# WeebLabs/DSPi

Measured on NVIDIA H100. Metric: audio samples/sec (whole box) at 65536ch x 10-band EQ, 96 kHz; % HBM roofline, higher is better.
Workload: dtype f32

## Files before the change

dspi_b200/csrc/engine.cu:

```cuda
#include <cstdarg>
#include <cstdio>
#include <cstdlib>
#include <cstring>
#include <algorithm>
#include <new>
#include <utility>
#include <vector>
#include <sched.h>
#include <unistd.h>
#include <sys/syscall.h>

#include "eq_kernels.cuh"
#include "eq_jit.h"

namespace {

thread_local char g_err[512] = "";

int fail(int code, const char *fmt, ...)
{
    va_list ap;
    va_start(ap, fmt);
    vsnprintf(g_err, sizeof(g_err), fmt, ap);
    va_end(ap);
// ... 143 lines not shown
    int ndev = 0;
    if (cudaGetDeviceCount(&ndev) != cudaSuccess || ndev == 0) { cudaGetLastError(); return fail(DSPI_ENODEV, "no CUDA device (there is no CPU fallback)"); }
    if (desc->device < 0 || desc->device >= ndev) return fail(DSPI_ENODEV, "device %d out of range (%d visible)", desc->device, ndev);
    int major = 0;
    CU_OK(cudaDeviceGetAttribute(&major, cudaDevAttrComputeCapabilityMajor, desc->device));
    if (major != 9) return fail(DSPI_ENODEV, "device %d has compute capability %d.x; the kernels are built for sm_90a only", desc->device, major);
    if (!encode_fn()) return fail(DSPI_ENODEV, "driver does not export cuTensorMapEncodeTiled");
    CU_OK(cudaSetDevice(desc->device));

    dspi_eq *e = new (std::nothrow) dspi_eq();
    if (!e) return fail(DSPI_ENOMEM, "host allocation failed");
    memset(e, 0, sizeof(*e));
    e->desc = *desc;
    e->sig_dirty = true;
    const bool q28 = desc->arith == DSPI_ARITH_Q28;
    e->cpl = 2;
    if (const char *v = getenv("DSPI_F32_CPL")) e->cpl = atoi(v) == 1 ? 1 : 2;
    if (q28) e->cpl = 1;
    e->rows = 32u * e->cpl;
    e->n_groups = (desc->n_channels + e->rows - 1) / e->rows;
    e->c_pad = e->n_groups * e->rows;
    e->aos_elem = q28 ? sizeof(dspi_biquad_q28) : sizeof(dspi_biquad_f32);

    cudaError_t err;
    const size_t aos_bytes = (size_t)e->c_pad * DSPI_MAX_BANDS * e->aos_elem;
    const size_t coef_bytes = q28 ? (size_t)e->n_groups * DSPI_MAX_BANDS * 20 * 32 * 4 : (size_t)e->c_pad * DSPI_MAX_BANDS * 8 * 4;
    if ((err = cudaStreamCreateWithFlags(&e->stream, cudaStreamNonBlocking)) != cudaSuccess) goto cuda_fail;
    if ((err = cudaStreamCreateWithFlags(&e->s_h2d, cudaStreamNonBlocking)) != cudaSuccess) goto cuda_fail;
    if ((err = cudaStreamCreateWithFlags(&e->s_d2h, cudaStreamNonBlocking)) != cudaSuccess) goto cuda_fail;
    if ((err = cudaEventCreateWithFlags(&e->ev_begin, cudaEventDisableTiming)) != cudaSuccess) goto cuda_fail;
    for (int i = 0; i < kHostBufs; i++) {
        if ((err = cudaStreamCreateWithFlags(&e->s_k[i], cudaStreamNonBlocking)) != cudaSuccess) goto cuda_fail;
// ... 133 lines not shown
    const cuuint64_t gstride[1] = { (cuuint64_t)ld * 4 };
    const cuuint32_t box[2] = { 32, e->rows };
    const cuuint32_t estr[2] = { 1, 1 };
    const CUtensorMapDataType dt = e->desc.arith == DSPI_ARITH_Q28 ? CU_TENSOR_MAP_DATA_TYPE_INT32 : CU_TENSOR_MAP_DATA_TYPE_FLOAT32;
    CUresult r = encode_fn()(out, dt, 2, d_samples, gdim, gstride, box, estr, CU_TENSOR_MAP_INTERLEAVE_NONE, CU_TENSOR_MAP_SWIZZLE_128B,
                             CU_TENSOR_MAP_L2_PROMOTION_L2_256B, CU_TENSOR_MAP_FLOAT_OOB_FILL_NONE);
    if (r != CUDA_SUCCESS) return fail(DSPI_ECUDA, "cuTensorMapEncodeTiled failed (%d) for T=%u ld=%u rows=%u", (int)r, T, ld, n_rows);
    return DSPI_OK;
}

static int refresh_kernel_choice(dspi_eq *e)
{
    e->sig_dirty = false;
    e->jit = nullptr;
    if (e->desc.arith == DSPI_ARITH_Q28) { snprintf(e->kinfo, sizeof(e->kinfo), "aot q28 cascade (K2)"); return DSPI_OK; }
    if (e->cpl != 2) { snprintf(e->kinfo, sizeof(e->kinfo), "aot scalar generic (DSPI_F32_CPL=1)"); return DSPI_OK; }
    const uint32_t C = e->desc.n_channels, nb = e->desc.n_bands;
    const int nbt = nb <= 10 ? 10 : 12;
    const uint32_t step = C > 2048 ? C / 2048 : 1;
    const uint32_t cnt = (C + step - 1) / step;
    std::vector<uint64_t> w(cnt);
    CU_OK(cudaMemcpy2DAsync(w.data(), 8, e->d_modes_eff ? e->d_modes_eff : e->d_modes, (size_t)step * 8, 8, cnt, cudaMemcpyDeviceToHost, e->stream));
    CU_OK(cudaStreamSynchronize(e->stream));
    const uint64_t mask = (1ull << (4 * nb)) - 1;
    for (auto &x : w) x &= mask;
    std::vector<uint64_t> sorted(w);
    std::sort(sorted.begin(), sorted.end());
    uint64_t best = 0;
    uint32_t best_n = 0;
    for (uint32_t i = 0; i < cnt;) {
        uint32_t j = i;
        while (j < cnt && sorted[j] == sorted[i]) j++;
        if (j - i > best_n) { best_n = j - i; best = sorted[i]; }
        i = j;
    }
    uint64_t tdf2 = 0;
    for (int b = 0; b < nbt; b++) tdf2 |= (uint64_t)dspi::kModeTdf2 << (4 * b);
    const unsigned pct = (unsigned)(100ull * best_n / cnt);
    if (best == tdf2 && (int)nb == nbt) {
        snprintf(e->kinfo, sizeof(e->kinfo), "aot straight-line biquad (%u%% of sampled channels are all-TDF2)", pct);
        return DSPI_OK;
    }
    bool force = false;
    const bool on = dspi::jit::enabled_by_env(&force);
    const char *why = nullptr;
    if (!on) why = "DSPI_JIT=0";
    else if (best == 0) why = "all bands bypassed";
    else if (2 * best_n < cnt) why = "no dominant topology vector";
    else if (!force && C < 1024) why = "engine below 1024 channels (DSPI_JIT=force overrides)";
    if (why) {
        snprintf(e->kinfo, sizeof(e->kinfo), "aot generic column path (%s)", why);
        return DSPI_OK;
    }
    char msg[256] = "";
    e->jit = dspi::jit::acquire(best, e->desc.arith == DSPI_ARITH_F32_FUSED, nbt, e->desc.device, msg, sizeof(msg));
    if (e->jit) snprintf(e->kinfo, sizeof(e->kinfo), "jit sig=0x%llx nb=%d (%u%% of sampled channels)", (unsigned long long)best, nbt, pct);
    else snprintf(e->kinfo, sizeof(e->kinfo), "aot generic column path (jit unavailable: %.200s)", msg);
    return DSPI_OK;
}

static int launch_eq(dspi_eq *e, void *d_samples, uint32_t T, uint32_t ld, uint32_t g0, uint32_t ng, uint32_t n_rows, cudaStream_t stream)
{
    dspi::EqLaunch a;
    memset(&a, 0, sizeof(a));
    const bool tma_ok = (ld % 4 == 0) && (((uintptr_t)d_samples & 15) == 0);
    if (tma_ok) {
        if (e->tm_ptr != d_samples || e->tm_T != T || e->tm_ld != ld || e->tm_rows != n_rows) {
            int rc = make_tmap(e, d_samples, T, ld, n_rows, &e->tmap);
            if (rc) return rc;
            e->tm_ptr = d_samples; e->tm_T = T; e->tm_ld = ld; e->tm_rows = n_rows;
        }
        a.tmap = e->tmap;
// ... 21 lines not shown
    if (q28) err = dspi::launch_eq_q28(a, stream);
    else if (e->jit && !(a.dbg & 12u)) {
        char msg[200] = "";
        err = dspi::jit::launch(e->jit, a, stream, msg, sizeof(msg));
        if (err != cudaSuccess) return fail(DSPI_ECUDA, "%s", msg);
    } else err = dspi::launch_eq_f32(a, e->desc.arith == DSPI_ARITH_F32_FUSED, e->cpl, stream);
    if (err != cudaSuccess) return fail(DSPI_ECUDA, "EQ kernel launch: %s", cudaGetErrorString(err));
    e->launches++;
    return DSPI_OK;
}

}

namespace dspi {

void *eq_aos_mirror(dspi_eq *e) { return e->d_aos; }

static int remask(dspi_eq *e, cudaStream_t s)
{
    if (!e->d_skip) return DSPI_OK;
    if (e->desc.arith == DSPI_ARITH_Q28) {
        CU_OK(launch_skip_q28((int32_t *)e->d_coef, e->d_skip, e->desc.n_channels, s));
        e->launches++;
        return DSPI_OK;
    }
    if (!e->d_modes_eff) {
        CU_OK(cudaMalloc(&e->d_modes_eff, (size_t)e->c_pad * 8));
        CU_OK(cudaMemsetAsync(e->d_modes_eff, 0, (size_t)e->c_pad * 8, s));
    }
    CU_OK(launch_mask_modes(e->d_modes, e->d_skip, e->d_modes_eff, e->desc.n_channels, s));
// ... 52 lines not shown
int eq_state_imported(dspi_eq *e, cudaStream_t s)
{
    e->sig_dirty = true;
    return remask(e, s);
}

int eq_process_on(dspi_eq *e, void *d_samples, uint32_t T, uint32_t ld, cudaStream_t s)
{
    if (T == 0) return DSPI_OK;
    return launch_eq(e, d_samples, T, ld, 0, e->n_groups, e->desc.n_channels, s);
}

int eq_process_range_on(dspi_eq *e, void *d_rows, uint32_t T, uint32_t ld, uint32_t ch0, uint32_t n, cudaStream_t s)
{
    if (T == 0 || n == 0) return DSPI_OK;
    if (ch0 % e->rows) return fail(DSPI_EINVAL, "first channel %u is not a multiple of the engine's group size %u", ch0, e->rows);
    CU_OK(cudaSetDevice(e->desc.device));
    return launch_eq(e, d_rows, T, ld, ch0 / e->rows, (n + e->rows - 1) / e->rows, n, s);
}

}

extern "C" {

int dspi_eq_kernel_info(dspi_eq *e, char *buf, size_t cap)
{
    if (!e || !buf || cap == 0) return fail(DSPI_EINVAL, "null argument");
    CU_OK(cudaSetDevice(e->desc.device));
    if (e->sig_dirty) {
        int rc = refresh_kernel_choice(e);
        if (rc) return rc;
// ... 5 lines not shown
int dspi_eq_process_device(dspi_eq *e, void *d_samples, uint32_t T, uint32_t ld)
{
    if (!e || !d_samples) return fail(DSPI_EINVAL, "null argument");
    if (T == 0) return DSPI_OK;
    if (ld < T) return fail(DSPI_EINVAL, "row stride %u < T %u", ld, T);
    CU_OK(cudaSetDevice(e->desc.device));
    return launch_eq(e, d_samples, T, ld, 0, e->n_groups, e->desc.n_channels, e->stream);
}

int dspi_eq_process_device_range(dspi_eq *e, void *d_rows, uint32_t T, uint32_t ld, uint32_t ch0, uint32_t n)
{
    if (!e || !d_rows) return fail(DSPI_EINVAL, "null argument");
    if (T == 0 || n == 0) return DSPI_OK;
    if (ld < T) return fail(DSPI_EINVAL, "row stride %u < T %u", ld, T);
    if ((uint64_t)ch0 + n > e->desc.n_channels) return fail(DSPI_ERANGE, "channels [%u, %u) outside engine of %u", ch0, ch0 + n, e->desc.n_channels);
    if (ch0 % e->rows) return fail(DSPI_EINVAL, "first channel %u is not a multiple of the engine's group size %u", ch0, e->rows);
    CU_OK(cudaSetDevice(e->desc.device));
    return launch_eq(e, d_rows, T, ld, ch0 / e->rows, (n + e->rows - 1) / e->rows, n, e->stream);
}

}

namespace dspi {
int eq_process_remote_enqueue(dspi_eq *e, void *remote, uint32_t T, uint32_t ch0, uint32_t n_ch)
{
    if (T == 0 || n_ch == 0) return DSPI_OK;
    CU_OK(cudaSetDevice(e->desc.device));
    const uint32_t ld = (T + 3) & ~3u;
    static const size_t chunk_mb_env = [] { const char *v = getenv("DSPI_HOST_CHUNK_MB"); const long n = v ? atol(v) : 0; return (size_t)(n >= 1 && n <= 1024 ? n : 0); }();
    cudaPointerAttributes pa;
    const bool on_device = cudaPointerGetAttributes(&pa, remote) == cudaSuccess && pa.type == cudaMemoryTypeDevice;
// ... 76 lines not shown
```

dspi_b200/csrc/eq_core.cuh:

```cuda
#pragma once
#include "eq_modes.cuh"

namespace dspi {
namespace core {

constexpr int kSub = 8;

struct P2 { unsigned long long v; };

__device__ __forceinline__ float v_mul(float a, float b) { return __fmul_rn(a, b); }
__device__ __forceinline__ float v_add(float a, float b) { return __fadd_rn(a, b); }
__device__ __forceinline__ float v_fma(float a, float b, float c) { return __fmaf_rn(a, b, c); }
__device__ __forceinline__ P2 v_mul(P2 a, P2 b)
{
    P2 r;
    asm("{\n\t.reg .f32 a0, a1, b0, b1;\n\t"
        "mov.b64 {a0, a1}, %1;\n\tmov.b64 {b0, b1}, %2;\n\t"
        "mul.rn.ftz.f32 a0, a0, b0;\n\tmul.rn.ftz.f32 a1, a1, b1;\n\t"
        "mov.b64 %0, {a0, a1};\n\t}" : "=l"(r.v) : "l"(a.v), "l"(b.v));
    return r;
}
__device__ __forceinline__ P2 v_add(P2 a, P2 b)
{
    P2 r;
// ... 240 lines not shown

    __device__ __forceinline__ void store(V *base, bool shared_state = false) const
    {
#pragma unroll
        for (int b = 0; b < NB; b++) {
            if (shared_state) {
                st_cg(base + (b * 8 + 6) * 32, st[b][0]);
                st_cg(base + (b * 8 + 7) * 32, st[b][1]);
            } else {
                base[(b * 8 + 6) * 32] = st[b][0];
                base[(b * 8 + 7) * 32] = st[b][1];
            }
        }
    }

    __device__ __forceinline__ void run(V (&x)[kSub], int nvalid, const V nz)
    {
        if (all_tdf2 && nvalid == kSub) {
            V y[kSub];
#pragma unroll
            for (int b = 0; b < NB; b += 2) {
                tdf2_tile<FUSED>(x, y, c[b], st[b][0], st[b][1], nz);
                tdf2_tile<FUSED>(y, x, c[b + 1], st[b + 1][0], st[b + 1][1], nz);
            }
            return;
        }
        V y[kSub];
#pragma unroll
        for (int b = 0; b < NB; b++) {
            V(&in)[kSub] = (b & 1) ? y : x;
            V(&out)[kSub] = (b & 1) ? x : y;
            const uint32_t m = (b < (int)nb_active) ? ((uint32_t)(mode_w >> (4 * b)) & 15u) : kModeBypass;
            const bool fast = (((uni >> b) & 1u) || b >= (int)nb_active) && nvalid == kSub;
            if (fast) {
                if (m == kModeTdf2) tdf2_tile<FUSED>(in, out, c[b], st[b][0], st[b][1], nz);
                else if (m == kModeSvfPK) svf_tile<FUSED, kMixPK>(in, out, c[b], st[b][0], st[b][1], nz);
                else if (m == kModeSvfSH) svf_tile<FUSED, kMixSH>(in, out, c[b], st[b][0], st[b][1], nz);
                else if (m == kModeSvfLP) svf_tile<FUSED, kMixLP>(in, out, c[b], st[b][0], st[b][1], nz);
                else if (m == kModeSvfHP) svf_tile<FUSED, kMixHP>(in, out, c[b], st[b][0], st[b][1], nz);
                else {
#pragma unroll
                    for (int i = 0; i < kSub; i++) out[i] = in[i];
                }
            } else {
                float xs[CPL][kSub], ns0[CPL], ns1[CPL];
#pragma unroll
                for (int h = 0; h < CPL; h++) {
#pragma unroll
                    for (int i = 0; i < kSub; i++) xs[h][i] = Lanes<V>::get(in[i], h);
                    const uint32_t mh = (uint32_t)(mode_h[h] >> (4 * b)) & 15u;
                    const float2 ns = slow_band<FUSED>(xs[h], nvalid, mh, Lanes<V>::get(c[b][0], h), Lanes<V>::get(c[b][1], h),
                                                       Lanes<V>::get(c[b][2], h), Lanes<V>::get(c[b][3], h), Lanes<V>::get(c[b][4], h),
                                                       Lanes<V>::get(c[b][5], h), Lanes<V>::get(st[b][0], h), Lanes<V>::get(st[b][1], h));
                    ns0[h] = ns.x;
                    ns1[h] = ns.y;
                }
                v_make(st[b][0], ns0);
                v_make(st[b][1], ns1);
#pragma unroll
                for (int i = 0; i < kSub; i++) {
                    float part[CPL];
#pragma unroll
                    for (int h = 0; h < CPL; h++) part[h] = xs[h][i];
                    v_make(out[i], part);
                }
            }
        }
        static_assert(NB % 2 == 0, "results must land back in x");
    }

    template <unsigned long long W, int B, bool IN_X>
    __device__ __forceinline__ void sig_from(V (&x)[kSub], V (&y)[kSub], const V nz)
    {
        if constexpr (B < NB) {
            constexpr uint32_t m = (uint32_t)((W >> (4 * B)) & 15ull);
            V(&in)[kSub] = IN_X ? x : y;
            V(&out)[kSub] = IN_X ? y : x;
            if constexpr (m == kModeBypass) {
                sig_from<W, B + 1, IN_X>(x, y, nz);
            } else {
                if constexpr (m == kModeTdf2) tdf2_tile<FUSED>(in, out, c[B], st[B][0], st[B][1], nz);
                else svf_tile<FUSED, (int)m>(in, out, c[B], st[B][0], st[B][1], nz);
                sig_from<W, B + 1, !IN_X>(x, y, nz);
            }
        } else if constexpr (!IN_X) {
#pragma unroll
            for (int i = 0; i < kSub; i++) x[i] = y[i];
        }
    }
    template <unsigned long long W>
    __device__ __forceinline__ bool sig_match() const
    {
        bool mine = true;
#pragma unroll
        for (int h = 0; h < CPL; h++) mine = mine && mode_h[h] == W;
        return __all_sync(0xffffffffu, mine);
    }
    template <unsigned long long W>
    __device__ __forceinline__ void run_sig(V (&x)[kSub], const V nz)
    {
        V y[kSub];
        sig_from<W, 0, true>(x, y, nz);
    }

    template <int MODE>
    __device__ __forceinline__ void band_loop(V *col, int n, const V (&cc)[6], V &s0, V &s1, const V nz)
    {
#pragma unroll 2
        for (int i = 0; i < n; i += 4) {
            V x[4], y[4];
#pragma unroll
            for (int j = 0; j < 4; j++) x[j] = col[(i + j) * 32];
            if constexpr (MODE == (int)kModeTdf2) tdf2_tile<FUSED>(x, y, cc, s0, s1, nz);
            else svf_tile<FUSED, MODE>(x, y, cc, s0, s1, nz);
#pragma unroll
            for (int j = 0; j < 4; j++) col[(i + j) * 32] = y[j];
// ... 76 lines not shown
```

dspi_b200/csrc/eq_f32.cu:

```cuda
#include "eq_kernels.cuh"
#include "eq_f32_kernel.cuh"

namespace dspi {
namespace {

using namespace core;
using k1::kStages;
using k1::kTileT;

template <typename V, bool FUSED, int NB, bool DYN>
__global__ void __launch_bounds__(256 * 2 / Lanes<V>::CPL, 1)
eq_f32_kernel(const __grid_constant__ CUtensorMap tmap, float *__restrict__ samples, uint32_t ld, V *__restrict__ coef,
              const uint64_t *__restrict__ modes, uint32_t n_groups, uint32_t n_rows, uint32_t T, uint32_t nb_active, uint32_t use_tma, uint32_t dbg,
              unsigned long long nz_bits, uint32_t slice_tiles, uint32_t *__restrict__ sched)
{
    k1::eq_f32_body<V, FUSED, NB, DYN, k1::NoSig>(tmap, samples, ld, coef, modes, n_groups, n_rows, T, nb_active, use_tma, dbg, nz_bits, slice_tiles, sched);
}

template <typename V, bool FUSED, int NB>
cudaError_t launch_one(const EqLaunch &a, cudaStream_t stream)
{
    constexpr int CPL = Lanes<V>::CPL;
    constexpr int kWarps = 16 / CPL;
    constexpr size_t smem = (size_t)kWarps * kStages * (32 * CPL) * kTileT * 4;
    auto kern = eq_f32_kernel<V, FUSED, NB, false>;
    auto kern_dyn = eq_f32_kernel<V, FUSED, NB, true>;
    static PerDeviceOnce once;
    int dev = 0;
    if (once.needs(&dev)) {
        cudaError_t e = cudaFuncSetAttribute(kern, cudaFuncAttributeMaxDynamicSharedMemorySize, (int)smem);
        if (e == cudaSuccess) e = cudaFuncSetAttribute(kern_dyn, cudaFuncAttributeMaxDynamicSharedMemorySize, (int)smem);
        if (e != cudaSuccess) return e;
        once.mark(dev);
    }
    const uint32_t n_groups = a.n_groups;
    uint32_t grid = (n_groups + kWarps - 1) / kWarps;
    uint32_t slice_tiles = 0;
    uint32_t *sched = nullptr;
    const uint32_t ntiles = (a.T + kTileT - 1) / kTileT;
    if (a.sched && a.use_tma && ntiles >= 32 && (a.dbg & 8u)) {
        slice_tiles = 16;
        sched = a.sched;
        if (grid > (uint32_t)a.n_sms) grid = a.n_sms;
        else if (grid < (uint32_t)a.n_sms && (uint32_t)a.n_sms * kWarps <= n_groups * ((ntiles + slice_tiles - 1) / slice_tiles)) grid = a.n_sms;
        cudaError_t e = cudaMemsetAsync(sched, 0, (size_t)(1 + n_groups) * sizeof(uint32_t), stream);
        if (e != cudaSuccess) return e;
    }
    if (sched)
        kern_dyn<<<grid, kWarps * 32, smem, stream>>>(a.tmap, (float *)a.samples, a.ld, (V *)a.coef, a.modes, n_groups, a.n_rows, a.T, a.n_bands, a.use_tma,
                                                      a.dbg, 0x8000000080000000ull, slice_tiles, sched);
    else
        kern<<<grid, kWarps * 32, smem, stream>>>(a.tmap, (float *)a.samples, a.ld, (V *)a.coef, a.modes, n_groups, a.n_rows, a.T, a.n_bands, a.use_tma,
                                                  a.dbg, 0x8000000080000000ull, 0u, nullptr);
    return cudaGetLastError();
}

// ... 88 lines not shown
```

dspi_b200/csrc/eq_f32_jit_entry.cuh:

```cuda
#include "eq_f32_kernel.cuh"

#ifndef DSPI_JIT_NB
#define DSPI_JIT_NB 10
#endif

extern "C" __global__ void __launch_bounds__(256, 1)
eq_f32_jit(const __grid_constant__ CUtensorMap tmap, float *__restrict__ samples, uint32_t ld, dspi::core::P2 *__restrict__ coef,
           const uint64_t *__restrict__ modes, uint32_t n_groups, uint32_t n_rows, uint32_t T, uint32_t nb_active, uint32_t use_tma, uint32_t dbg,
           unsigned long long nz_bits, uint32_t slice_tiles, uint32_t *__restrict__ sched)
{
    dspi::k1::eq_f32_body<dspi::core::P2, (DSPI_JIT_FUSED) != 0, DSPI_JIT_NB, false, dspi::k1::SigWord<(DSPI_JIT_SIG)>>(
        tmap, samples, ld, coef, modes, n_groups, n_rows, T, nb_active, use_tma, dbg, nz_bits, slice_tiles, sched);
}
```

dspi_b200/csrc/eq_f32_kernel.cuh:

```cuda
#pragma once
#include "eq_core.cuh"

namespace dspi {
namespace k1 {

using namespace core;

constexpr int kTileT = 32;
constexpr int kStages = 3;

struct NoSig { static constexpr bool enabled = false; static constexpr unsigned long long word = 0; };
template <unsigned long long W> struct SigWord { static constexpr bool enabled = true; static constexpr unsigned long long word = W; };

template <typename V, bool FUSED, int NB, bool DYN, typename SIG>
__device__ __forceinline__ void eq_f32_body(const CUtensorMap &tmap, float *__restrict__ samples, uint32_t ld, V *__restrict__ coef,
              const uint64_t *__restrict__ modes, uint32_t n_groups, uint32_t n_rows, uint32_t T, uint32_t nb_active, uint32_t use_tma, uint32_t dbg, unsigned long long nz_bits, uint32_t slice_tiles, uint32_t *__restrict__ sched)
{
    constexpr int CPL = Lanes<V>::CPL;
    constexpr int kRows = 32 * CPL;
    constexpr int kWarps = 16 / CPL;
    constexpr uint32_t kStageBytes = kRows * kTileT * 4;

    extern __shared__ __align__(1024) uint8_t smem_raw[];
    __shared__ uint64_t bars[16 / Lanes<V>::CPL][kStages];

    const int warp = threadIdx.x >> 5, lane = threadIdx.x & 31;

    uint8_t *my_smem = smem_raw + (size_t)warp * kStages * kStageBytes;
    uint64_t *full = bars[warp];
    if (lane == 0) {
        if (use_tma) prefetch_tmap(&tmap);
        for (int s = 0; s < kStages; s++) mbar_init(&full[s], 1);
        fence_mbar_init();
    }
    __syncwarp();

    const V nz = v_bits<V>(nz_bits);
    const uint32_t ntiles = (T + kTileT - 1) / kTileT;
    const bool mem_on = !(dbg & 2u);
    const uint32_t sw = (lane & 7) << 4;

    const uint32_t n_slices = DYN ? (ntiles + slice_tiles - 1) / slice_tiles : 1;
    const uint32_t n_items = DYN ? n_groups * n_slices : 0;
    uint32_t tcount = 0;
    for (;;) {
        uint32_t g, tile_begin, tile_end, slice = 0;
        if constexpr (DYN) {
            uint32_t item = 0;
            if (lane == 0) item = atomicAdd(&sched[0], 1u);
            item = __shfl_sync(0xffffffffu, item, 0);
            if (item >= n_items) break;
            slice = item / n_groups;
            g = item - slice * n_groups;
            tile_begin = slice * slice_tiles;
            tile_end = min(ntiles, tile_begin + slice_tiles);
// ... 1 lines not shown
                if (lane == 0) {
                    const volatile uint32_t *flag = sched + 1 + g;
                    while (*flag < slice) __nanosleep(100);
                    __threadfence();
                }
                __syncwarp();
            }
        } else {
            g = blockIdx.x * kWarps + warp;
            if (g >= n_groups) break;
            tile_begin = 0;
            tile_end = ntiles;
        }
        const int c0 = g * kRows;

        auto issue_load = [&](uint32_t tile, uint32_t seq) {
            const uint32_t s = seq % kStages;
            mbar_arrive_expect_tx(&full[s], kStageBytes);
            tma_load_2d(my_smem + s * kStageBytes, &tmap, &full[s], tile * kTileT, c0);
        };
        if (use_tma && mem_on && lane == 0) {
            if constexpr (DYN) tma_store_wait_read<0>();
            for (uint32_t j = 0; j + 1 < kStages && tile_begin + j < tile_end; j++) issue_load(tile_begin + j, tcount + j);
        }

        EqBank<V, FUSED, NB> bank;
        V *my_coef = coef + (size_t)g * kMaxBands * 8 * 32 + lane;
        {
            const uint64_t *mp[CPL];
#pragma unroll
            for (int h = 0; h < CPL; h++) mp[h] = modes + (size_t)g * kRows + h * 32 + lane;
            bank.load(my_coef, mp, nb_active, DYN);
        }
        bool straight = bank.all_tdf2;
        if constexpr (SIG::enabled) straight = bank.template sig_match<SIG::word>();

        for (uint32_t tile = tile_begin; tile < tile_end; tile++, tcount++) {
            const uint32_t s = tcount % kStages;
            uint8_t *buf = my_smem + s * kStageBytes;
            if (use_tma) {
                if (mem_on) mbar_wait(&full[s], (tcount / kStages) & 1);
            } else {
                const uint32_t t = tile * kTileT + lane;
                for (int r = 0; r < kRows; r++) {
                    const uint32_t ch = c0 + r;
                    float v = 0.0f;
                    if (t < T && ch < n_rows) v = samples[(size_t)ch * ld + t];
                    *reinterpret_cast<float *>(buf + r * 128 + ((((lane >> 2) << 4) ^ ((r & 7) << 4)) | ((lane & 3) << 2))) = v;
                }
                __syncwarp();
            }

            const int tile_valid = min((int)kTileT, (int)(T - tile * kTileT));
            if (straight && tile_valid == kTileT && !(dbg & 4u)) {
    #pragma unroll 1
                for (int sub = 0; sub < kTileT / kSub; sub++) {
                    V x[kSub];
                    float4 q[CPL][2];
    #pragma unroll
                    for (int h = 0; h < CPL; h++) {
                        const uint8_t *row = buf + (lane + 32 * h) * 128;
                        q[h][0] = *reinterpret_cast<const float4 *>(row + (((2 * sub) << 4) ^ sw));
                        q[h][1] = *reinterpret_cast<const float4 *>(row + (((2 * sub + 1) << 4) ^ sw));
                    }
    #pragma unroll
                    for (int i = 0; i < kSub; i++) {
                        float part[CPL];
    #pragma unroll
                        for (int h = 0; h < CPL; h++) {
                            const float4 &qq = q[h][i >> 2];
                            part[h] = (i & 3) == 0 ? qq.x : (i & 3) == 1 ? qq.y : (i & 3) == 2 ? qq.z : qq.w;
                        }
                        v_make(x[i], part);
                    }
                    if (!(dbg & 1u)) {
                        if constexpr (SIG::enabled) bank.template run_sig<SIG::word>(x, nz);
                        else bank.run(x, kSub, nz);
                    }
    #pragma unroll
                    for (int h = 0; h < CPL; h++) {
                        uint8_t *row = buf + (lane + 32 * h) * 128;
                        *reinterpret_cast<float4 *>(row + (((2 * sub) << 4) ^ sw)) =
                            make_float4(Lanes<V>::get(x[0], h), Lanes<V>::get(x[1], h), Lanes<V>::get(x[2], h), Lanes<V>::get(x[3], h));
                        *reinterpret_cast<float4 *>(row + (((2 * sub + 1) << 4) ^ sw)) =
                            make_float4(Lanes<V>::get(x[4], h), Lanes<V>::get(x[5], h), Lanes<V>::get(x[6], h), Lanes<V>::get(x[7], h));
                    }
                }
            } else {
                float4 q[CPL][8];
    #pragma unroll
                for (int h = 0; h < CPL; h++) {
                    const uint8_t *row = buf + (lane + 32 * h) * 128;
    #pragma unroll
                    for (int k = 0; k < 8; k++) q[h][k] = *reinterpret_cast<const float4 *>(row + ((k << 4) ^ sw));
                }
                __syncwarp();
                V *col = reinterpret_cast<V *>(buf) + lane;
    #pragma unroll
                for (int n = 0; n < kTileT; n++) {
                    float part[CPL];
    #pragma unroll
                    for (int h = 0; h < CPL; h++) {
                        const float4 &qq = q[h][n >> 2];
                        part[h] = (n & 3) == 0 ? qq.x : (n & 3) == 1 ? qq.y : (n & 3) == 2 ? qq.z : qq.w;
                    }
                    V v;
                    v_make(v, part);
                    col[n * 32] = v;
                }
                if (!(dbg & 1u)) bank.run_columns(col, tile_valid, nz);
                float back[CPL][kTileT];
    #pragma unroll
                for (int n = 0; n < kTileT; n++) {
                    const V v = col[n * 32];
    #pragma unroll
                    for (int h = 0; h < CPL; h++) back[h][n] = Lanes<V>::get(v, h);
                }
                __syncwarp();
    #pragma unroll
                for (int h = 0; h < CPL; h++) {
                    uint8_t *row = buf + (lane + 32 * h) * 128;
    #pragma unroll
                    for (int k = 0; k < 8; k++)
                        *reinterpret_cast<float4 *>(row + ((k << 4) ^ sw)) = make_float4(back[h][4 * k], back[h][4 * k + 1], back[h][4 * k + 2], back[h][4 * k + 3]);
                }
            }

            if (use_tma) {
                fence_proxy_async_smem();
                __syncwarp();
                if (lane == 0 && mem_on) {
                    tma_store_2d(&tmap, buf, tile * kTileT, c0);
                    tma_store_commit();
                    const uint32_t nxt = tile + kStages - 1;
                    if (nxt < tile_end) {
                        tma_store_wait_read<1>();
                        issue_load(nxt, tcount + kStages - 1);
                    }
                }
            } else {
                __syncwarp();
                const uint32_t t = tile * kTileT + lane;
                for (int r = 0; r < kRows; r++) {
                    const uint32_t ch = c0 + r;
                    const float v = *reinterpret_cast<const float *>(buf + r * 128 + ((((lane >> 2) << 4) ^ ((r & 7) << 4)) | ((lane & 3) << 2)));
                    if (t < T && ch < n_rows) samples[(size_t)ch * ld + t] = v;
                }
                __syncwarp();
            }
        }


        bank.store(my_coef, DYN);
        if constexpr (!DYN) break;
        __threadfence();
        __syncwarp();
        if (lane == 0) atomicExch(&sched[1 + g], slice + 1);
    }
    if (use_tma && lane == 0) tma_store_wait_all<0>();
}

// ... 4 lines not shown
```

dspi_b200/csrc/eq_jit.cu:

```cuda
#include "eq_kernels.cuh"
#include "eq_f32_kernel.cuh"
#include "eq_jit.h"

#include <dlfcn.h>
#include <mutex>
#include <stdio.h>
#include <string.h>
#include <string>
#include <vector>

#include "jit_headers.inc"

namespace dspi {
namespace jit {
namespace {

typedef struct _nvrtcProgram *nvrtcProgram;
struct Nvrtc {
    void *so = nullptr;
    int (*CreateProgram)(nvrtcProgram *, const char *, const char *, int, const char *const *, const char *const *) = nullptr;
    int (*CompileProgram)(nvrtcProgram, int, const char *const *) = nullptr;
    int (*DestroyProgram)(nvrtcProgram *) = nullptr;
    int (*GetCUBINSize)(nvrtcProgram, size_t *) = nullptr;
    int (*GetCUBIN)(nvrtcProgram, char *) = nullptr;
// ... 54 lines not shown
}

std::string cu_err(CUresult r)
{
    const char *s = nullptr;
    if (driver().GetErrorString) driver().GetErrorString(r, &s);
    char b[96];
    snprintf(b, sizeof(b), "%s (%d)", s ? s : "CUDA driver error", (int)r);
    return b;
}

struct Entry {
    uint64_t sig;
    bool fused;
    int nb;
    CUlibrary lib;
    CUkernel kern;
    uint64_t smem_set;
    std::string fail;
};

std::mutex g_mu;
std::vector<Entry *> g_cache;

constexpr int kWarps = 8;
constexpr size_t kSmem = (size_t)kWarps * k1::kStages * 64 * k1::kTileT * 4;

Entry *compile(uint64_t sig, bool fused, int nb)
{
    Entry *en = new Entry{ sig, fused, nb, nullptr, nullptr, 0, "" };
    Nvrtc &n = nvrtc();
    Driver &d = driver();
    if (!n.ok) { en->fail = "libnvrtc not available"; return en; }
    if (!d.ok) { en->fail = "driver lacks cuLibraryLoadData/cuLibraryGetKernel"; return en; }
    nvrtcProgram prog = nullptr;
    int rc = n.CreateProgram(&prog, "#include \"eq_f32_jit_entry.cuh\"\n", "dspi_eq_jit.cu", kJitHeaderCount, kJitHeaderSrc, kJitHeaderNames);
    if (rc != 0) { en->fail = "nvrtcCreateProgram failed"; return en; }
    char dsig[64], dfused[32], dnb[32];
    snprintf(dsig, sizeof(dsig), "-DDSPI_JIT_SIG=0x%llxull", (unsigned long long)sig);
    snprintf(dfused, sizeof(dfused), "-DDSPI_JIT_FUSED=%d", fused ? 1 : 0);
    snprintf(dnb, sizeof(dnb), "-DDSPI_JIT_NB=%d", nb);
    const char *opts[] = { "--gpu-architecture=sm_90a", "-std=c++17", "-ftz=true", "-prec-div=true", "-prec-sqrt=true", "-fmad=false",
                           "-lineinfo", dsig, dfused, dnb };
    rc = n.CompileProgram(prog, (int)(sizeof(opts) / sizeof(opts[0])), opts);
    if (rc != 0) {
        size_t ls = 0;
        n.GetProgramLogSize(prog, &ls);
        std::string log(ls ? ls : 1, '\0');
        if (ls) n.GetProgramLog(prog, &log[0]);
        if (log.size() > 400) log.resize(400);
        en->fail = std::string("nvrtcCompileProgram: ") + (n.GetErrorString ? n.GetErrorString(rc) : "error") + ": " + log;
        n.DestroyProgram(&prog);
        return en;
    }
    size_t sz = 0;
    std::vector<char> cubin;
    if (n.GetCUBINSize(prog, &sz) != 0 || sz == 0) { en->fail = "nvrtcGetCUBINSize failed"; n.DestroyProgram(&prog); return en; }
    cubin.resize(sz);
// ... 6 lines not shown
    return en;
}

}

bool enabled_by_env(bool *force)
{
    *force = false;
    const char *v = getenv("DSPI_JIT");
    if (!v) return true;
    if (!strcmp(v, "0") || !strcmp(v, "off")) return false;
    if (!strcmp(v, "force") || !strcmp(v, "2")) *force = true;
    return true;
}

void *acquire(uint64_t sig, bool fused, int nb, int device, char *msg, size_t cap)
{
    std::lock_guard<std::mutex> lk(g_mu);
    Entry *en = nullptr;
    for (Entry *e : g_cache)
        if (e->sig == sig && e->fused == fused && e->nb == nb) { en = e; break; }
    if (!en) {
        en = compile(sig, fused, nb);
        g_cache.push_back(en);
    }
    if (!en->fail.empty()) {
        if (msg && cap) snprintf(msg, cap, "%s", en->fail.c_str());
        return nullptr;
    }
    if (device >= 0 && device < 64 && !((en->smem_set >> device) & 1)) {
        CUdevice dev = device;
        CUresult r = driver().KernelSetAttribute(CU_FUNC_ATTRIBUTE_MAX_DYNAMIC_SHARED_SIZE_BYTES, (int)kSmem, en->kern, dev);
        if (r != CUDA_SUCCESS) {
            if (msg && cap) snprintf(msg, cap, "cuKernelSetAttribute: %s", cu_err(r).c_str());
            return nullptr;
        }
        en->smem_set |= 1ull << device;
    }
// ... 27 lines not shown
```

dspi_b200/csrc/eq_jit.h:

```cpp
#pragma once
#include "eq_kernels.cuh"

namespace dspi {
namespace jit {

bool enabled_by_env(bool *force);

void *acquire(uint64_t sig, bool fused, int nb, int device, char *msg, size_t cap);

cudaError_t launch(void *handle, const EqLaunch &a, cudaStream_t stream, char *msg, size_t cap);

}
}
```

Measured before the change: 301.8 billion.

## Default to one channel per lane with 64-sample tiles split into two TMA boxes

Switches the default f32 geometry from two channels per lane (64 rows x 32 samples) to one channel per lane (32 rows x 64 samples). Each stage stays at 8 KB and is loaded and stored as two 128B-swizzled TMA boxes, and the sub-block length and JIT kernel now scale with the lanes-per-channel choice. The aim is more independent warps per channel block and a longer time run per tile, without the packed-pair arithmetic. In exchange there are twice as many TMA ops per stage, different register pressure, and the alignment needed for ranges changes.

```diff
diff --git a/dspi_b200/csrc/engine.cu b/dspi_b200/csrc/engine.cu
--- a/dspi_b200/csrc/engine.cu
+++ b/dspi_b200/csrc/engine.cu
@@ -181,8 +181,8 @@
     e->desc = *desc;
     e->sig_dirty = true;
     const bool q28 = desc->arith == DSPI_ARITH_Q28;
-    e->cpl = 2;
-    if (const char *v = getenv("DSPI_F32_CPL")) e->cpl = atoi(v) == 1 ? 1 : 2;
+    e->cpl = 1;
+    if (const char *v = getenv("DSPI_F32_CPL")) e->cpl = atoi(v) == 2 ? 2 : 1;
     if (q28) e->cpl = 1;
     e->rows = 32u * e->cpl;
     e->n_groups = (desc->n_channels + e->rows - 1) / e->rows;
@@ -346,7 +346,7 @@
     e->sig_dirty = false;
     e->jit = nullptr;
     if (e->desc.arith == DSPI_ARITH_Q28) { snprintf(e->kinfo, sizeof(e->kinfo), "aot q28 cascade (K2)"); return DSPI_OK; }
-    if (e->cpl != 2) { snprintf(e->kinfo, sizeof(e->kinfo), "aot scalar generic (DSPI_F32_CPL=1)"); return DSPI_OK; }
+    const char *geo = e->cpl == 1 ? "tile 32 rows x 64 samples, 1 ch/lane" : "tile 64 rows x 32 samples, 2 ch/lane";
     const uint32_t C = e->desc.n_channels, nb = e->desc.n_bands;
     const int nbt = nb <= 10 ? 10 : 12;
     const uint32_t step = C > 2048 ? C / 2048 : 1;
@@ -370,7 +370,7 @@
     for (int b = 0; b < nbt; b++) tdf2 |= (uint64_t)dspi::kModeTdf2 << (4 * b);
     const unsigned pct = (unsigned)(100ull * best_n / cnt);
     if (best == tdf2 && (int)nb == nbt) {
-        snprintf(e->kinfo, sizeof(e->kinfo), "aot straight-line biquad (%u%% of sampled channels are all-TDF2)", pct);
+        snprintf(e->kinfo, sizeof(e->kinfo), "aot straight-line biquad (%u%% of sampled channels are all-TDF2); %s", pct, geo);
         return DSPI_OK;
     }
     bool force = false;
@@ -381,13 +381,13 @@
     else if (2 * best_n < cnt) why = "no dominant topology vector";
     else if (!force && C < 1024) why = "engine below 1024 channels (DSPI_JIT=force overrides)";
     if (why) {
-        snprintf(e->kinfo, sizeof(e->kinfo), "aot generic column path (%s)", why);
+        snprintf(e->kinfo, sizeof(e->kinfo), "aot generic column path (%s); %s", why, geo);
         return DSPI_OK;
     }
     char msg[256] = "";
-    e->jit = dspi::jit::acquire(best, e->desc.arith == DSPI_ARITH_F32_FUSED, nbt, e->desc.device, msg, sizeof(msg));
-    if (e->jit) snprintf(e->kinfo, sizeof(e->kinfo), "jit sig=0x%llx nb=%d (%u%% of sampled channels)", (unsigned long long)best, nbt, pct);
-    else snprintf(e->kinfo, sizeof(e->kinfo), "aot generic column path (jit unavailable: %.200s)", msg);
+    e->jit = dspi::jit::acquire(best, e->desc.arith == DSPI_ARITH_F32_FUSED, nbt, e->cpl, e->desc.device, msg, sizeof(msg));
+    if (e->jit) snprintf(e->kinfo, sizeof(e->kinfo), "jit sig=0x%llx nb=%d (%u%% of sampled channels); %s", (unsigned long long)best, nbt, pct, geo);
+    else snprintf(e->kinfo, sizeof(e->kinfo), "aot generic column path (jit unavailable: %.200s); %s", msg, geo);
     return DSPI_OK;
 }
 
@@ -439,6 +439,8 @@
 
 namespace dspi {
 
+static uint32_t range_unit(const dspi_eq *e) { return e->desc.arith == DSPI_ARITH_Q28 ? e->rows : 64u; }
+
 void *eq_aos_mirror(dspi_eq *e) { return e->d_aos; }
 
 static int remask(dspi_eq *e, cudaStream_t s)
@@ -521,7 +523,7 @@
 int eq_process_range_on(dspi_eq *e, void *d_rows, uint32_t T, uint32_t ld, uint32_t ch0, uint32_t n, cudaStream_t s)
 {
     if (T == 0 || n == 0) return DSPI_OK;
-    if (ch0 % e->rows) return fail(DSPI_EINVAL, "first channel %u is not a multiple of the engine's group size %u", ch0, e->rows);
+    if (ch0 % range_unit(e)) return fail(DSPI_EINVAL, "first channel %u is not a multiple of %u", ch0, range_unit(e));
     CU_OK(cudaSetDevice(e->desc.device));
     return launch_eq(e, d_rows, T, ld, ch0 / e->rows, (n + e->rows - 1) / e->rows, n, s);
 }
@@ -557,7 +559,7 @@
     if (T == 0 || n == 0) return DSPI_OK;
     if (ld < T) return fail(DSPI_EINVAL, "row stride %u < T %u", ld, T);
     if ((uint64_t)ch0 + n > e->desc.n_channels) return fail(DSPI_ERANGE, "channels [%u, %u) outside engine of %u", ch0, ch0 + n, e->desc.n_channels);
-    if (ch0 % e->rows) return fail(DSPI_EINVAL, "first channel %u is not a multiple of the engine's group size %u", ch0, e->rows);
+    if (ch0 % dspi::range_unit(e)) return fail(DSPI_EINVAL, "first channel %u is not a multiple of %u", ch0, dspi::range_unit(e));
     CU_OK(cudaSetDevice(e->desc.device));
     return launch_eq(e, d_rows, T, ld, ch0 / e->rows, (n + e->rows - 1) / e->rows, n, e->stream);
 }
diff --git a/dspi_b200/csrc/eq_core.cuh b/dspi_b200/csrc/eq_core.cuh
--- a/dspi_b200/csrc/eq_core.cuh
+++ b/dspi_b200/csrc/eq_core.cuh
@@ -3,8 +3,6 @@
 
 namespace dspi {
 namespace core {
-
-constexpr int kSub = 8;
 
 struct P2 { unsigned long long v; };
 
@@ -278,10 +276,11 @@
         }
     }
 
-    __device__ __forceinline__ void run(V (&x)[kSub], int nvalid, const V nz)
-    {
-        if (all_tdf2 && nvalid == kSub) {
-            V y[kSub];
+    template <int N>
+    __device__ __forceinline__ void run(V (&x)[N], int nvalid, const V nz)
+    {
+        if (all_tdf2 && nvalid == N) {
+            V y[N];
 #pragma unroll
             for (int b = 0; b < NB; b += 2) {
                 tdf2_tile<FUSED>(x, y, c[b], st[b][0], st[b][1], nz);
@@ -289,13 +288,13 @@
             }
             return;
         }
-        V y[kSub];
+        V y[N];
 #pragma unroll
         for (int b = 0; b < NB; b++) {
-            V(&in)[kSub] = (b & 1) ? y : x;
-            V(&out)[kSub] = (b & 1) ? x : y;
+            V(&in)[N] = (b & 1) ? y : x;
+            V(&out)[N] = (b & 1) ? x : y;
             const uint32_t m = (b < (int)nb_active) ? ((uint32_t)(mode_w >> (4 * b)) & 15u) : kModeBypass;
-            const bool fast = (((uni >> b) & 1u) || b >= (int)nb_active) && nvalid == kSub;
+            const bool fast = (((uni >> b) & 1u) || b >= (int)nb_active) && nvalid == N;
             if (fast) {
                 if (m == kModeTdf2) tdf2_tile<FUSED>(in, out, c[b], st[b][0], st[b][1], nz);
                 else if (m == kModeSvfPK) svf_tile<FUSED, kMixPK>(in, out, c[b], st[b][0], st[b][1], nz);
@@ -304,14 +303,14 @@
                 else if (m == kModeSvfHP) svf_tile<FUSED, kMixHP>(in, out, c[b], st[b][0], st[b][1], nz);
                 else {
 #pragma unroll
-                    for (int i = 0; i < kSub; i++) out[i] = in[i];
-                }
-            } else {
-                float xs[CPL][kSub], ns0[CPL], ns1[CPL];
+                    for (int i = 0; i < N; i++) out[i] = in[i];
+                }
+            } else {
+                float xs[CPL][N], ns0[CPL], ns1[CPL];
 #pragma unroll
                 for (int h = 0; h < CPL; h++) {
 #pragma unroll
-                    for (int i = 0; i < kSub; i++) xs[h][i] = Lanes<V>::get(in[i], h);
+                    for (int i = 0; i < N; i++) xs[h][i] = Lanes<V>::get(in[i], h);
                     const uint32_t mh = (uint32_t)(mode_h[h] >> (4 * b)) & 15u;
                     const float2 ns = slow_band<FUSED>(xs[h], nvalid, mh, Lanes<V>::get(c[b][0], h), Lanes<V>::get(c[b][1], h),
                                                        Lanes<V>::get(c[b][2], h), Lanes<V>::get(c[b][3], h), Lanes<V>::get(c[b][4], h),
@@ -322,7 +321,7 @@
                 v_make(st[b][0], ns0);
                 v_make(st[b][1], ns1);
 #pragma unroll
-                for (int i = 0; i < kSub; i++) {
+                for (int i = 0; i < N; i++) {
                     float part[CPL];
 #pragma unroll
                     for (int h = 0; h < CPL; h++) part[h] = xs[h][i];
@@ -333,13 +332,13 @@
         static_assert(NB % 2 == 0, "results must land back in x");
     }
 
-    template <unsigned long long W, int B, bool IN_X>
-    __device__ __forceinline__ void sig_from(V (&x)[kSub], V (&y)[kSub], const V nz)
+    template <unsigned long long W, int B, bool IN_X, int N>
+    __device__ __forceinline__ void sig_from(V (&x)[N], V (&y)[N], const V nz)
     {
         if constexpr (B < NB) {
             constexpr uint32_t m = (uint32_t)((W >> (4 * B)) & 15ull);
-            V(&in)[kSub] = IN_X ? x : y;
-            V(&out)[kSub] = IN_X ? y : x;
+            V(&in)[N] = IN_X ? x : y;
+            V(&out)[N] = IN_X ? y : x;
             if constexpr (m == kModeBypass) {
                 sig_from<W, B + 1, IN_X>(x, y, nz);
             } else {
@@ -349,7 +348,7 @@
             }
         } else if constexpr (!IN_X) {
 #pragma unroll
-            for (int i = 0; i < kSub; i++) x[i] = y[i];
+            for (int i = 0; i < N; i++) x[i] = y[i];
         }
     }
     template <unsigned long long W>
@@ -360,10 +359,10 @@
         for (int h = 0; h < CPL; h++) mine = mine && mode_h[h] == W;
         return __all_sync(0xffffffffu, mine);
     }
-    template <unsigned long long W>
-    __device__ __forceinline__ void run_sig(V (&x)[kSub], const V nz)
-    {
-        V y[kSub];
+    template <unsigned long long W, int N>
+    __device__ __forceinline__ void run_sig(V (&x)[N], const V nz)
+    {
+        V y[N];
         sig_from<W, 0, true>(x, y, nz);
     }
 
diff --git a/dspi_b200/csrc/eq_f32.cu b/dspi_b200/csrc/eq_f32.cu
--- a/dspi_b200/csrc/eq_f32.cu
+++ b/dspi_b200/csrc/eq_f32.cu
@@ -5,11 +5,12 @@
 namespace {
 
 using namespace core;
+using k1::kStageBytes;
 using k1::kStages;
-using k1::kTileT;
+using k1::kWarps;
 
 template <typename V, bool FUSED, int NB, bool DYN>
-__global__ void __launch_bounds__(256 * 2 / Lanes<V>::CPL, 1)
+__global__ void __launch_bounds__(kWarps * 32, 1)
 eq_f32_kernel(const __grid_constant__ CUtensorMap tmap, float *__restrict__ samples, uint32_t ld, V *__restrict__ coef,
               const uint64_t *__restrict__ modes, uint32_t n_groups, uint32_t n_rows, uint32_t T, uint32_t nb_active, uint32_t use_tma, uint32_t dbg,
               unsigned long long nz_bits, uint32_t slice_tiles, uint32_t *__restrict__ sched)
@@ -20,9 +21,8 @@
 template <typename V, bool FUSED, int NB>
 cudaError_t launch_one(const EqLaunch &a, cudaStream_t stream)
 {
-    constexpr int CPL = Lanes<V>::CPL;
-    constexpr int kWarps = 16 / CPL;
-    constexpr size_t smem = (size_t)kWarps * kStages * (32 * CPL) * kTileT * 4;
+    constexpr int kTileT = k1::tile_t<V>();
+    constexpr size_t smem = (size_t)kWarps * kStages * kStageBytes;
     auto kern = eq_f32_kernel<V, FUSED, NB, false>;
     auto kern_dyn = eq_f32_kernel<V, FUSED, NB, true>;
     static PerDeviceOnce once;
@@ -38,8 +38,8 @@
     uint32_t slice_tiles = 0;
     uint32_t *sched = nullptr;
     const uint32_t ntiles = (a.T + kTileT - 1) / kTileT;
-    if (a.sched && a.use_tma && ntiles >= 32 && (a.dbg & 8u)) {
-        slice_tiles = 16;
+    if (a.sched && a.use_tma && a.T >= 1024 && (a.dbg & 8u)) {
+        slice_tiles = 512 / kTileT;
         sched = a.sched;
         if (grid > (uint32_t)a.n_sms) grid = a.n_sms;
         else if (grid < (uint32_t)a.n_sms && (uint32_t)a.n_sms * kWarps <= n_groups * ((ntiles + slice_tiles - 1) / slice_tiles)) grid = a.n_sms;
diff --git a/dspi_b200/csrc/eq_f32_jit_entry.cuh b/dspi_b200/csrc/eq_f32_jit_entry.cuh
--- a/dspi_b200/csrc/eq_f32_jit_entry.cuh
+++ b/dspi_b200/csrc/eq_f32_jit_entry.cuh
@@ -3,12 +3,17 @@
 #ifndef DSPI_JIT_NB
 #define DSPI_JIT_NB 10
 #endif
+#if DSPI_JIT_CPL == 2
+typedef dspi::core::P2 JitV;
+#else
+typedef float JitV;
+#endif
 
-extern "C" __global__ void __launch_bounds__(256, 1)
-eq_f32_jit(const __grid_constant__ CUtensorMap tmap, float *__restrict__ samples, uint32_t ld, dspi::core::P2 *__restrict__ coef,
+extern "C" __global__ void __launch_bounds__(dspi::k1::kWarps * 32, 1)
+eq_f32_jit(const __grid_constant__ CUtensorMap tmap, float *__restrict__ samples, uint32_t ld, JitV *__restrict__ coef,
            const uint64_t *__restrict__ modes, uint32_t n_groups, uint32_t n_rows, uint32_t T, uint32_t nb_active, uint32_t use_tma, uint32_t dbg,
            unsigned long long nz_bits, uint32_t slice_tiles, uint32_t *__restrict__ sched)
 {
-    dspi::k1::eq_f32_body<dspi::core::P2, (DSPI_JIT_FUSED) != 0, DSPI_JIT_NB, false, dspi::k1::SigWord<(DSPI_JIT_SIG)>>(
+    dspi::k1::eq_f32_body<JitV, (DSPI_JIT_FUSED) != 0, DSPI_JIT_NB, false, dspi::k1::SigWord<(DSPI_JIT_SIG)>>(
         tmap, samples, ld, coef, modes, n_groups, n_rows, T, nb_active, use_tma, dbg, nz_bits, slice_tiles, sched);
 }
diff --git a/dspi_b200/csrc/eq_f32_kernel.cuh b/dspi_b200/csrc/eq_f32_kernel.cuh
--- a/dspi_b200/csrc/eq_f32_kernel.cuh
+++ b/dspi_b200/csrc/eq_f32_kernel.cuh
@@ -6,8 +6,16 @@
 
 using namespace core;
 
-constexpr int kTileT = 32;
 constexpr int kStages = 3;
+constexpr int kWarps = 8;
+constexpr uint32_t kStageBytes = 8192;
+template <typename V> __host__ __device__ constexpr int tile_t() { return 64 / Lanes<V>::CPL; }
+template <typename V> __host__ __device__ constexpr int sub_t() { return tile_t<V>() / 4; }
+
+__device__ __forceinline__ uint32_t chunk_off(int r, int k, uint32_t half_bytes)
+{
+    return (uint32_t)(k >> 3) * half_bytes + r * 128 + ((((k & 7) ^ (r & 7))) << 4);
+}
 
 struct NoSig { static constexpr bool enabled = false; static constexpr unsigned long long word = 0; };
 template <unsigned long long W> struct SigWord { static constexpr bool enabled = true; static constexpr unsigned long long word = W; };
@@ -18,11 +26,14 @@
 {
     constexpr int CPL = Lanes<V>::CPL;
     constexpr int kRows = 32 * CPL;
-    constexpr int kWarps = 16 / CPL;
-    constexpr uint32_t kStageBytes = kRows * kTileT * 4;
+    constexpr int kTileT = tile_t<V>();
+    constexpr int kSub = sub_t<V>();
+    constexpr int kHalves = kTileT / 32;
+    constexpr uint32_t kHalfBytes = kRows * 128;
+    static_assert(kRows * kTileT * 4 == (int)kStageBytes, "every geometry fills the same 8 KB stage");
 
     extern __shared__ __align__(1024) uint8_t smem_raw[];
-    __shared__ uint64_t bars[16 / Lanes<V>::CPL][kStages];
+    __shared__ uint64_t bars[kWarps][kStages];
 
     const int warp = threadIdx.x >> 5, lane = threadIdx.x & 31;
 
@@ -38,7 +49,6 @@
     const V nz = v_bits<V>(nz_bits);
     const uint32_t ntiles = (T + kTileT - 1) / kTileT;
     const bool mem_on = !(dbg & 2u);
-    const uint32_t sw = (lane & 7) << 4;
 
     const uint32_t n_slices = DYN ? (ntiles + slice_tiles - 1) / slice_tiles : 1;
     const uint32_t n_items = DYN ? n_groups * n_slices : 0;
@@ -70,10 +80,13 @@
         }
         const int c0 = g * kRows;
 
+        auto n_boxes = [&](uint32_t tile) { return kHalves == 1 || tile * kTileT + 32 < T ? kHalves : 1; };
         auto issue_load = [&](uint32_t tile, uint32_t seq) {
             const uint32_t s = seq % kStages;
-            mbar_arrive_expect_tx(&full[s], kStageBytes);
-            tma_load_2d(my_smem + s * kStageBytes, &tmap, &full[s], tile * kTileT, c0);
+            const int nb = n_boxes(tile);
+            mbar_arrive_expect_tx(&full[s], nb * kHalfBytes);
+            for (int h = 0; h < nb; h++)
+                tma_load_2d(my_smem + s * kStageBytes + h * kHalfBytes, &tmap, &full[s], tile * kTileT + h * 32, c0);
         };
         if (use_tma && mem_on && lane == 0) {
             if constexpr (DYN) tma_store_wait_read<0>();
@@ -97,28 +110,30 @@
             if (use_tma) {
                 if (mem_on) mbar_wait(&full[s], (tcount / kStages) & 1);
             } else {
-                const uint32_t t = tile * kTileT + lane;
                 for (int r = 0; r < kRows; r++) {
                     const uint32_t ch = c0 + r;
-                    float v = 0.0f;
-                    if (t < T && ch < n_rows) v = samples[(size_t)ch * ld + t];
-                    *reinterpret_cast<float *>(buf + r * 128 + ((((lane >> 2) << 4) ^ ((r & 7) << 4)) | ((lane & 3) << 2))) = v;
+                    for (int h = 0; h < kHalves; h++) {
+                        const uint32_t t = tile * kTileT + h * 32 + lane;
+                        float v = 0.0f;
+                        if (t < T && ch < n_rows) v = samples[(size_t)ch * ld + t];
+                        *reinterpret_cast<float *>(buf + chunk_off(r, h * 8 + (lane >> 2), kHalfBytes) + ((lane & 3) << 2)) = v;
+                    }
                 }
                 __syncwarp();
             }
 
             const int tile_valid = min((int)kTileT, (int)(T - tile * kTileT));
-            if (straight && tile_valid == kTileT && !(dbg & 4u)) {
+            if (straight && tile_valid % kSub == 0 && !(dbg & 4u)) {
     #pragma unroll 1
-                for (int sub = 0; sub < kTileT / kSub; sub++) {
+                for (int sub = 0; sub < tile_valid / kSub; sub++) {
+                    constexpr int kQ = kSub / 4;
                     V x[kSub];
-                    float4 q[CPL][2];
-    #pragma unroll
-                    for (int h = 0; h < CPL; h++) {
-                        const uint8_t *row = buf + (lane + 32 * h) * 128;
-                        q[h][0] = *reinterpret_cast<const float4 *>(row + (((2 * sub) << 4) ^ sw));
-                        q[h][1] = *reinterpret_cast<const float4 *>(row + (((2 * sub + 1) << 4) ^ sw));
-                    }
+                    float4 q[CPL][kQ];
+    #pragma unroll
+                    for (int h = 0; h < CPL; h++)
+    #pragma unroll
+                        for (int j = 0; j < kQ; j++)
+                            q[h][j] = *reinterpret_cast<const float4 *>(buf + chunk_off(lane + 32 * h, kQ * sub + j, kHalfBytes));
     #pragma unroll
                     for (int i = 0; i < kSub; i++) {
                         float part[CPL];
@@ -134,22 +149,19 @@
                         else bank.run(x, kSub, nz);
                     }
     #pragma unroll
-                    for (int h = 0; h < CPL; h++) {
-                        uint8_t *row = buf + (lane + 32 * h) * 128;
-                        *reinterpret_cast<float4 *>(row + (((2 * sub) << 4) ^ sw)) =
-                            make_float4(Lanes<V>::get(x[0], h), Lanes<V>::get(x[1], h), Lanes<V>::get(x[2], h), Lanes<V>::get(x[3], h));
-                        *reinterpret_cast<float4 *>(row + (((2 * sub + 1) << 4) ^ sw)) =
-                            make_float4(Lanes<V>::get(x[4], h), Lanes<V>::get(x[5], h), Lanes<V>::get(x[6], h), Lanes<V>::get(x[7], h));
-                    }
+                    for (int h = 0; h < CPL; h++)
+    #pragma unroll
+                        for (int j = 0; j < kQ; j++)
+                            *reinterpret_cast<float4 *>(buf + chunk_off(lane + 32 * h, kQ * sub + j, kHalfBytes)) =
+                                make_float4(Lanes<V>::get(x[4 * j], h), Lanes<V>::get(x[4 * j + 1], h), Lanes<V>::get(x[4 * j + 2], h),
+                                            Lanes<V>::get(x[4 * j + 3], h));
                 }
             } else {
-                float4 q[CPL][8];
-    #pragma unroll
-                for (int h = 0; h < CPL; h++) {
-                    const uint8_t *row = buf + (lane + 32 * h) * 128;
-    #pragma unroll
-                    for (int k = 0; k < 8; k++) q[h][k] = *reinterpret_cast<const float4 *>(row + ((k << 4) ^ sw));
-                }
+                float4 q[CPL][kTileT / 4];
+    #pragma unroll
+                for (int h = 0; h < CPL; h++)
+    #pragma unroll
+                    for (int k = 0; k < kTileT / 4; k++) q[h][k] = *reinterpret_cast<const float4 *>(buf + chunk_off(lane + 32 * h, k, kHalfBytes));
                 __syncwarp();
                 V *col = reinterpret_cast<V *>(buf) + lane;
     #pragma unroll
@@ -174,19 +186,19 @@
                 }
                 __syncwarp();
     #pragma unroll
-                for (int h = 0; h < CPL; h++) {
-                    uint8_t *row = buf + (lane + 32 * h) * 128;
-    #pragma unroll
-                    for (int k = 0; k < 8; k++)
-                        *reinterpret_cast<float4 *>(row + ((k << 4) ^ sw)) = make_float4(back[h][4 * k], back[h][4 * k + 1], back[h][4 * k + 2], back[h][4 * k + 3]);
-                }
+                for (int h = 0; h < CPL; h++)
+    #pragma unroll
+                    for (int k = 0; k < kTileT / 4; k++)
+                        *reinterpret_cast<float4 *>(buf + chunk_off(lane + 32 * h, k, kHalfBytes)) =
+                            make_float4(back[h][4 * k], back[h][4 * k + 1], back[h][4 * k + 2], back[h][4 * k + 3]);
             }
 
             if (use_tma) {
                 fence_proxy_async_smem();
                 __syncwarp();
                 if (lane == 0 && mem_on) {
-                    tma_store_2d(&tmap, buf, tile * kTileT, c0);
+                    const int nb = n_boxes(tile);
+                    for (int h = 0; h < nb; h++) tma_store_2d(&tmap, buf + h * kHalfBytes, tile * kTileT + h * 32, c0);
                     tma_store_commit();
                     const uint32_t nxt = tile + kStages - 1;
                     if (nxt < tile_end) {
@@ -196,11 +208,13 @@
                 }
             } else {
                 __syncwarp();
-                const uint32_t t = tile * kTileT + lane;
                 for (int r = 0; r < kRows; r++) {
                     const uint32_t ch = c0 + r;
-                    const float v = *reinterpret_cast<const float *>(buf + r * 128 + ((((lane >> 2) << 4) ^ ((r & 7) << 4)) | ((lane & 3) << 2)));
-                    if (t < T && ch < n_rows) samples[(size_t)ch * ld + t] = v;
+                    for (int h = 0; h < kHalves; h++) {
+                        const uint32_t t = tile * kTileT + h * 32 + lane;
+                        const float v = *reinterpret_cast<const float *>(buf + chunk_off(r, h * 8 + (lane >> 2), kHalfBytes) + ((lane & 3) << 2));
+                        if (t < T && ch < n_rows) samples[(size_t)ch * ld + t] = v;
+                    }
                 }
                 __syncwarp();
             }
diff --git a/dspi_b200/csrc/eq_jit.cu b/dspi_b200/csrc/eq_jit.cu
--- a/dspi_b200/csrc/eq_jit.cu
+++ b/dspi_b200/csrc/eq_jit.cu
@@ -92,6 +92,7 @@
     uint64_t sig;
     bool fused;
     int nb;
+    int cpl;
     CUlibrary lib;
     CUkernel kern;
     uint64_t smem_set;
@@ -101,12 +102,12 @@
 std::mutex g_mu;
 std::vector<Entry *> g_cache;
 
-constexpr int kWarps = 8;
-constexpr size_t kSmem = (size_t)kWarps * k1::kStages * 64 * k1::kTileT * 4;
-
-Entry *compile(uint64_t sig, bool fused, int nb)
-{
-    Entry *en = new Entry{ sig, fused, nb, nullptr, nullptr, 0, "" };
+constexpr int kWarps = k1::kWarps;
+constexpr size_t kSmem = (size_t)kWarps * k1::kStages * k1::kStageBytes;
+
+Entry *compile(uint64_t sig, bool fused, int nb, int cpl)
+{
+    Entry *en = new Entry{ sig, fused, nb, cpl, nullptr, nullptr, 0, "" };
     Nvrtc &n = nvrtc();
     Driver &d = driver();
     if (!n.ok) { en->fail = "libnvrtc not available"; return en; }
@@ -114,12 +115,13 @@
     nvrtcProgram prog = nullptr;
     int rc = n.CreateProgram(&prog, "#include \"eq_f32_jit_entry.cuh\"\n", "dspi_eq_jit.cu", kJitHeaderCount, kJitHeaderSrc, kJitHeaderNames);
     if (rc != 0) { en->fail = "nvrtcCreateProgram failed"; return en; }
-    char dsig[64], dfused[32], dnb[32];
+    char dsig[64], dfused[32], dnb[32], dcpl[32];
     snprintf(dsig, sizeof(dsig), "-DDSPI_JIT_SIG=0x%llxull", (unsigned long long)sig);
     snprintf(dfused, sizeof(dfused), "-DDSPI_JIT_FUSED=%d", fused ? 1 : 0);
     snprintf(dnb, sizeof(dnb), "-DDSPI_JIT_NB=%d", nb);
+    snprintf(dcpl, sizeof(dcpl), "-DDSPI_JIT_CPL=%d", cpl);
     const char *opts[] = { "--gpu-architecture=sm_90a", "-std=c++17", "-ftz=true", "-prec-div=true", "-prec-sqrt=true", "-fmad=false",
-                           "-lineinfo", dsig, dfused, dnb };
+                           "-lineinfo", dsig, dfused, dnb, dcpl };
     rc = n.CompileProgram(prog, (int)(sizeof(opts) / sizeof(opts[0])), opts);
     if (rc != 0) {
         size_t ls = 0;
@@ -156,14 +158,14 @@
     return true;
 }
 
-void *acquire(uint64_t sig, bool fused, int nb, int device, char *msg, size_t cap)
+void *acquire(uint64_t sig, bool fused, int nb, int cpl, int device, char *msg, size_t cap)
 {
     std::lock_guard<std::mutex> lk(g_mu);
     Entry *en = nullptr;
     for (Entry *e : g_cache)
-        if (e->sig == sig && e->fused == fused && e->nb == nb) { en = e; break; }
+        if (e->sig == sig && e->fused == fused && e->nb == nb && e->cpl == cpl) { en = e; break; }
     if (!en) {
-        en = compile(sig, fused, nb);
+        en = compile(sig, fused, nb, cpl);
         g_cache.push_back(en);
     }
     if (!en->fail.empty()) {
diff --git a/dspi_b200/csrc/eq_jit.h b/dspi_b200/csrc/eq_jit.h
--- a/dspi_b200/csrc/eq_jit.h
+++ b/dspi_b200/csrc/eq_jit.h
@@ -6,7 +6,7 @@
 
 bool enabled_by_env(bool *force);
 
-void *acquire(uint64_t sig, bool fused, int nb, int device, char *msg, size_t cap);
+void *acquire(uint64_t sig, bool fused, int nb, int cpl, int device, char *msg, size_t cap);
 
 cudaError_t launch(void *handle, const EqLaunch &a, cudaStream_t stream, char *msg, size_t cap);
 
```

New measurement: 337.8 billion, median of 6. 11.9% higher.
